# Meng-333/FastDiffSR

Measured on AMD Instinct MI355X. Metric: 256x256 SR images/sec at T=20, higher is better.
Workload: dtype f16x3; 1 GPU; x4 64->256, batch=16/GPU, T=20, random-init FastDiffSR UNet (inner 64, mults 1-2-4-4), 256x256, conv arithmetic f16x3 (BASELINE configs[1]); batch_per_gpu=16, global_batch=16, noise=drawn in the loop by the engine (Philox4x32-10), hipgraph=False, parallelism=dp1 (independent batches, weights broadcast once)

## Files before the change

fastdiffsr_amd/csrc/fdsr_conv_k32.hip:

```cpp
#include "fdsr_kernels.h"
#include "fdsr_act_io.h"

#include <type_traits>

namespace fdsr {

typedef float k_f32x4 __attribute__((ext_vector_type(4)));
typedef _Float16 k_h8 __attribute__((ext_vector_type(8)));
typedef _Float16 k_h4 __attribute__((ext_vector_type(4)));
typedef __bf16 k_b8 __attribute__((ext_vector_type(8)));
typedef __bf16 k_b4 __attribute__((ext_vector_type(4)));

__device__ __forceinline__ float silu_k(float v) { return v * __builtin_amdgcn_rcpf(1.0f + __expf(-v)); }

#ifndef XS_F16X3
#define XS_F16X3 2
#endif
#ifndef XS_BF16
#define XS_BF16 4
#endif
#ifndef K32_PIN
#define K32_PIN 1
#endif
#ifndef K32_RIDER2
#define K32_RIDER2 1
#endif
#ifndef K32_SPLIT
#define K32_SPLIT 1
#endif
#ifndef K32_SPLIT_BF16
#define K32_SPLIT_BF16 1
#endif
#ifndef K32_MIXSPLIT
#define K32_MIXSPLIT 1
#endif
#ifndef K32_PEEL
#define K32_PEEL 1
#endif
#ifndef K32_GNB_DIAG
#define K32_GNB_DIAG 0
#endif
#ifndef K32_DIAG
#define K32_DIAG 0
#endif
#ifndef K32_RFIRST
#define K32_RFIRST 1
#endif
#ifndef K32_PIN16
#define K32_PIN16 0
#endif

constexpr int K32_GNC_MAXC = 1024, K32_GNC_MAXP = K32_GNC_MAXC / 2 + 32, K32_GNC_LDS = K32_GNC_MAXP * 32 + K32_GNC_MAXC * 8;

template <int TH, int WN, int PREC, int NW_ = 8>
struct ConvK32Cfg {
  static constexpr int TW = 32, NW = NW_, KC = 32;
  static constexpr int NP = PREC == PREC_F16X3 ? 2 : 1;
  static constexpr int WNP = PREC == PREC_BF16 ? 1 : 2;
  static constexpr int ROWB = 64 * NP;
  static constexpr int HH = TH + 2, HWD = TW + 2, NPIX = HH * HWD;
  static constexpr int WM = NW / WN, BN = 32 * WN, MB = TH / WM;
  static constexpr int NT = 64 * NW;
  static constexpr int Q4 = KC / 4;
  static constexpr int RPP = NT / Q4;
  static constexpr int NIN = (NPIX + RPP - 1) / RPP;
  static constexpr int BUF_BYTES = NPIX * ROWB;
  static constexpr int LDS_BYTES = 2 * BUF_BYTES;
  static constexpr int R = 3;
  static constexpr int XS = PREC == PREC_F16X3 ? XS_F16X3 : (NW_ == 4 && TH == 8 ? 3 : XS_BF16);
  static_assert(MB == 4 || MB == 3 || MB == 2, "wave tile = 4 (small grids: 2; small workgroups in f16x3: 3) rows of 32 pixels");
  static_assert(((TH - WM + 2) * HWD + 16) * ROWB < 65536, "fragment offsets must fit the ds_read immediate");
};

template <int PREC>
__device__ __forceinline__ int k32_slot(int slot, int hx) {
  return PREC == PREC_F16X3 ? (slot ^ (hx & 7)) : (slot ^ ((hx >> 1) & 3));
}

template <int TH, int WN, int PREC, bool RIDER, int NW = 8, bool RF = (NW == 4), bool GNB = false, bool DROP = false, bool GNC = false>
__global__ void __launch_bounds__(64 * NW, 2) conv_k32_kernel(const ConvParams p) {
  using Cfg = ConvK32Cfg<TH, WN, PREC, NW>;
  constexpr int TW = Cfg::TW, KC = Cfg::KC, NP = Cfg::NP, ROWB = Cfg::ROWB, HWD = Cfg::HWD, NPIX = Cfg::NPIX;
  constexpr int WM = Cfg::WM, BN = Cfg::BN, MB = Cfg::MB, RPP = Cfg::RPP, NIN = Cfg::NIN, R = Cfg::R, XS = Cfg::XS;
  constexpr bool PIN = TH == 16 ? K32_PIN16 != 0 : K32_PIN != 0;

  extern __shared__ __attribute__((aligned(16))) unsigned char smem_k[];
  unsigned char* sBuf0 = smem_k;
  unsigned char* sBuf1 = smem_k + Cfg::BUF_BYTES;
  const int Cin = p.C0 + p.C1;

  const int tid = threadIdx.x, lane = tid & 63, wave = tid >> 6;
  const int wn = wave % WN, wm = wave / WN;
  const int c15 = lane & 15, g = lane >> 4;

  const int nco = p.Cout_pad / BN;
  const int tilesX = (p.Wout + TW - 1) / TW, tilesY = (p.Hout + TH - 1) / TH;
  int bid;
  {
    const int nwg = gridDim.x, b = blockIdx.x;
    const int q8 = nwg >> 3, r8 = nwg & 7, xcd = b & 7, k = b >> 3;
    bid = (xcd < r8 ? xcd * (q8 + 1) : r8 * (q8 + 1) + (xcd - r8) * q8) + k;
  }
  const int SK = p.ksplit > 1 ? p.ksplit : 1;
  const int ksi = bid % SK;
  bid /= SK;
  const int cot = bid % nco;
  int pt = bid / nco;
  const int tx = pt % tilesX;
  pt /= tilesX;
  const int ty = pt % tilesY;
  const int n = pt / tilesY;
  const int oy0 = ty * TH, ox0 = tx * TW, co0 = cot * BN;

  const bool gn = GNC ? true : p.gn_scale != nullptr;

  if (NW == 4 && p.stagger > 0) {
    unsigned hwid;
    asm volatile("s_getreg_b32 %0, hwreg(HW_REG_HW_ID)" : "=s"(hwid));
    if ((hwid >> 16) & 1u) {
      const int n64 = p.stagger * (p.Cin_pad / KC + (RIDER ? p.nkr / 2 : 0));
      for (int i = 0; i < n64; i += 8) __builtin_amdgcn_s_sleep(8);
    }
  }

  const int q = tid & 7, row0 = tid >> 3;
  int in_pix[NIN];
  unsigned long long skeys = 0;
  static_assert(NIN <= 21, "swizzle keys are packed into one register pair");
#pragma unroll
  for (int i = 0; i < NIN; ++i) {
    const int pix = row0 + i * RPP;
    int v = -2;
    if (pix < NPIX) {
      const int hy = pix / HWD, hx = pix % HWD;
      const int iy = oy0 - 1 + hy, ix = ox0 - 1 + hx;
      const bool ok = iy >= 0 && iy < p.Hin && ix >= 0 && ix < p.Win;
      v = ok ? (n * p.Hin + iy) * p.Win + ix : -1;
      skeys |= (unsigned long long)k32_slot<PREC>(0, hx) << (3 * i);
    }
    in_pix[i] = v;
  }
  const int sbase = row0 * ROWB + 8 * (q & 1);

  using IO = ActIO<PREC>;
  typedef typename IO::Quad Quad;
  struct QM { Quad q; unsigned m; };
  constexpr bool RFIRST = RIDER && RF && K32_RFIRST != 0;
  constexpr bool SPLIT = K32_SPLIT != 0 && (PREC == PREC_F16X3 || K32_SPLIT_BF16 != 0) && (!RIDER || RFIRST);
  static_assert(!RFIRST || SPLIT, "the rider-first path writes whole chunks into rr1, which is sized for them only when SPLIT");
  constexpr int NA = SPLIT ? (NIN + 1) / 2 : NIN;
  typedef std::integral_constant<int, 0> I_0;
  typedef std::integral_constant<int, NA> I_A;
  typedef std::integral_constant<int, NIN> I_N;
  QM rin[NA];
  QM rr1[RIDER && SPLIT ? NIN : 1];
  QM rin2[RIDER && K32_RIDER2 && NW == 8 ? NIN : 1];
  k_f32x4 rsc = {1.f, 1.f, 1.f, 1.f}, rsh = {0.f, 0.f, 0.f, 0.f};
  const int nk = p.Cin_pad / KC;
  const int nk16 = p.Cin_pad / 16;
  const int nkr = RIDER ? p.nkr / 2 : 0;
  double* gnc_pr = reinterpret_cast<double*>(smem_k + Cfg::LDS_BYTES);
  float* gnc_sc = reinterpret_cast<float*>(smem_k + Cfg::LDS_BYTES + K32_GNC_MAXP * 32);
  float* gnc_sh = gnc_sc + K32_GNC_MAXC;
  int gnc_lo = 0, gnc_hi = 0, gnc_cpg = 1, gnc_q0 = 0, gnc_q1 = 0;
  constexpr int GNC_PT = (2 * K32_GNC_MAXP + Cfg::NT - 1) / Cfg::NT;
  uint4 gnc_ld[GNC ? GNC_PT : 1][GSUM_SHARDS / 2];
  constexpr int GNC_CT = (K32_GNC_MAXC + Cfg::NT - 1) / Cfg::NT;
  float gnc_gam[GNC ? GNC_CT : 1], gnc_bet[GNC ? GNC_CT : 1];
  auto gnc_issue = [&](int c_lo, int c_hi) __attribute__((always_inline)) {
    gnc_lo = c_lo; gnc_hi = c_hi;
    gnc_cpg = Cin / p.gs_G;
    gnc_q0 = (c_lo / gnc_cpg) * gnc_cpg / 2;
    gnc_q1 = ((c_hi - 1) / gnc_cpg + 1) * gnc_cpg / 2;
#pragma unroll
    for (int j = 0; j < GNC_PT; ++j) {
      const int u = tid + j * Cfg::NT, qc = min(gnc_q0 + (u >> 1), gnc_q1 - 1);
      const bool first = qc < (p.C0 >> 1);
      const unsigned long long* tab = first ? p.gs0 : p.gs1;
      const int np = (first ? p.C0 : p.C1) >> 1, ql = first ? qc : qc - (p.C0 >> 1);
#pragma unroll
      for (int sdx = 0; sdx < GSUM_SHARDS / 2; ++sdx)
        gnc_ld[j][sdx] = *reinterpret_cast<const uint4*>(tab + (((size_t)n * GSUM_SHARDS + (u & 1) * (GSUM_SHARDS / 2) + sdx) * np + ql) * 2);
    }
#pragma unroll
    for (int j = 0; j < GNC_CT; ++j) {
      const int cc = min(c_lo + tid + j * Cfg::NT, c_hi - 1);
      gnc_gam[j] = p.gs_gamma[cc];
      gnc_bet[j] = p.gs_beta[cc];
    }
  };
  auto gnc_finish = [&]() __attribute__((always_inline)) {
#pragma unroll
    for (int j = 0; j < GNC_PT; ++j) {
      const int u = tid + j * Cfg::NT, qi = gnc_q0 + (u >> 1);
      long long a = 0, b = 0;
#pragma unroll
      for (int sdx = 0; sdx < GSUM_SHARDS / 2; ++sdx) {
        a += (long long)(((unsigned long long)gnc_ld[j][sdx].y << 32) | gnc_ld[j][sdx].x);
        b += (long long)(((unsigned long long)gnc_ld[j][sdx].w << 32) | gnc_ld[j][sdx].z);
      }
      if (qi < gnc_q1) {
        gnc_pr[2 * u] = (double)a * (1.0 / (double)(1 << GSUM_BITS1));
        gnc_pr[2 * u + 1] = (double)b * (1.0 / (double)(1 << GSUM_BITS2));
      }
    }
    __syncthreads();
    const double inv = 1.0 / ((double)gnc_cpg * (double)p.Hin * (double)p.Win);
#pragma unroll
    for (int j = 0; j < GNC_CT; ++j) {
      const int c = gnc_lo + tid + j * Cfg::NT;
      if (c >= gnc_hi) break;
      const int g = c / gnc_cpg, hp = gnc_cpg >> 1;
      double s1 = 0.0, s2 = 0.0;
      for (int k = 0; k < 2 * hp; ++k) { s1 += gnc_pr[2 * (2 * (g * hp - gnc_q0) + k)]; s2 += gnc_pr[2 * (2 * (g * hp - gnc_q0) + k) + 1]; }
      const double mean = s1 * inv;
      double var = s2 * inv - mean * mean;
      var = var < 0.0 ? 0.0 : var;
      const double rstd = 1.0 / sqrt(var + (double)p.gs_eps);
      const float scv = (float)rstd * gnc_gam[j];
      gnc_sc[c - gnc_lo] = scv;
      gnc_sh[c - gnc_lo] = gnc_bet[j] - (float)mean * scv;
    }
    __syncthreads();
  };
  auto prefetch_rng = [&](int kc, QM* rin, auto i0_tag, auto i1_tag, bool load_gn) __attribute__((always_inline)) {
    constexpr int I0 = decltype(i0_tag)::value, I1 = decltype(i1_tag)::value;
    int cbase = kc * KC;
    const float* base;
    int Cs, cc;
    bool gg = gn;
    if (RIDER && kc >= nk) {
      cbase -= nk * KC;
      gg = false;
      if (cbase < p.Cr0) { base = p.xr0; Cs = p.Cr0; cc = cbase + q * 4; }
      else { base = p.xr1; Cs = p.Cr1; cc = cbase - p.Cr0 + q * 4; }
    } else if (cbase < p.C0) { base = p.x0; Cs = p.C0; cc = cbase + q * 4; }
    else { base = p.x1; Cs = p.C1; cc = cbase - p.C0 + q * 4; }
    if (!GNC && gg && load_gn) {
      rsc = *reinterpret_cast<const k_f32x4*>(p.gn_scale + (size_t)n * Cin + cbase + q * 4);
      rsh = *reinterpret_cast<const k_f32x4*>(p.gn_shift + (size_t)n * Cin + cbase + q * 4);
    }
#pragma unroll
    for (int i = I0; i < I1; ++i) {
      const size_t pi = (size_t)(in_pix[i] < 0 ? 0 : in_pix[i]);
      rin[i - I0].q = IO::load4(base, pi * Cs + cc);
      if (DROP)
        rin[i - I0].m = *reinterpret_cast<const unsigned*>(p.drop_mask + ((RIDER && kc >= nk) ? (size_t)0 : pi * Cs + cc));
    }
  };
  auto prefetch_to = [&](int kc, QM* rin) __attribute__((always_inline)) { prefetch_rng(kc, rin, I_0{}, I_N{}, true); };
  auto stage_rng = [&](int kc, unsigned char* buf, const QM* rin, auto i0_tag, auto i1_tag) __attribute__((always_inline)) {
    constexpr int I0 = decltype(i0_tag)::value, I1 = decltype(i1_tag)::value;
    k_f32x4 sc = rsc, sh = rsh;
    if (GNC && !(RIDER && kc >= nk)) {
      sc = *reinterpret_cast<const k_f32x4*>(gnc_sc + (kc * KC - gnc_lo + q * 4));
      sh = *reinterpret_cast<const k_f32x4*>(gnc_sh + (kc * KC - gnc_lo + q * 4));
    }
#pragma unroll
    for (int i = I0; i < I1; ++i) {
      if (NIN * RPP > NPIX && i == NIN - 1 && row0 + i * RPP >= NPIX) continue;
      k_f32x4 v = IO::widen(rin[i - I0].q);
      if (K32_DIAG & 16) v = sc;
      if ((K32_DIAG & 1) && gn) {
        v = v + sh;
      } else if (gn && !(RIDER && kc >= nk)) {
        v = v * sc + sh;
        if (!p.gn_plain) { v.x = silu_k(v.x); v.y = silu_k(v.y); v.z = silu_k(v.z); v.w = silu_k(v.w); }
        if (DROP) {
          const unsigned m = rin[i - I0].m;
#pragma unroll
          for (int e = 0; e < 4; ++e) v[e] *= (float)((m >> (8 * e)) & 0xffu) * p.drop_scale;
        }
      } else if (PREC == PREC_F16X3 && p.sat_flag) {
        sat_check(p.sat_flag, v, 65504.f);
      }
      const int sd = sbase + i * (RPP * ROWB) + 16 * ((q >> 1) ^ (int)((skeys >> (3 * i)) & 7u));
      unsigned char* dst = buf + sd;
      if (PREC == PREC_F16X3) {
        const float lim = in_pix[i] >= 0 ? 65504.f : 0.f;
#pragma unroll
        for (int e = 0; e < 4; ++e) v[e] = __builtin_amdgcn_fmed3f(v[e], -lim, lim);
#if K32_MIXSPLIT
        typedef _Float16 h2t __attribute__((ext_vector_type(2)));
        uint2 hi, lo;
        {
          const h2t h0 = {(_Float16)v[0], (_Float16)v[1]}, h1 = {(_Float16)v[2], (_Float16)v[3]};
          hi.x = __builtin_bit_cast(unsigned, h0);
          hi.y = __builtin_bit_cast(unsigned, h1);
        }
        asm("v_fma_mixlo_f16 %0, %1, -1.0, %2 op_sel:[0,0,0] op_sel_hi:[1,0,0]" : "=v"(lo.x) : "v"(hi.x), "v"(v[0]));
        asm("v_fma_mixhi_f16 %0, %1, -1.0, %2 op_sel:[1,0,0] op_sel_hi:[1,0,0]" : "+v"(lo.x) : "v"(hi.x), "v"(v[1]));
        asm("v_fma_mixlo_f16 %0, %1, -1.0, %2 op_sel:[0,0,0] op_sel_hi:[1,0,0]" : "=v"(lo.y) : "v"(hi.y), "v"(v[2]));
        asm("v_fma_mixhi_f16 %0, %1, -1.0, %2 op_sel:[1,0,0] op_sel_hi:[1,0,0]" : "+v"(lo.y) : "v"(hi.y), "v"(v[3]));
        *reinterpret_cast<uint2*>(dst) = hi;
        *reinterpret_cast<uint2*>(buf + (sd ^ 64)) = lo;
#else
        k_h4 hi = {(_Float16)v.x, (_Float16)v.y, (_Float16)v.z, (_Float16)v.w};
        k_h4 lo = {(_Float16)(v.x - (float)hi.x), (_Float16)(v.y - (float)hi.y), (_Float16)(v.z - (float)hi.z),
                   (_Float16)(v.w - (float)hi.w)};
        *reinterpret_cast<k_h4*>(dst) = hi;
        *reinterpret_cast<k_h4*>(buf + (sd ^ 64)) = lo;
#endif
      } else {
        const float keep = in_pix[i] >= 0 ? 1.f : 0.f;
        v = v * keep;
        const uint2 hb = stage4_16<PREC>(v);
        if (K32_DIAG & 8) asm volatile("" ::"v"(hb.x), "v"(hb.y));
        else *reinterpret_cast<uint2*>(dst) = hb;
      }
    }
  };
  auto stage_from = [&](int kc, unsigned char* buf, const QM* rin) __attribute__((always_inline)) { stage_rng(kc, buf, rin, I_0{}, I_N{}); };

  const uint4* wq = reinterpret_cast<const uint4*>(p.wq);
  const int nkt = RIDER ? nk + nkr : nk;
  uint4 Wf[R][2][NP];
  const int wlane = 32 * (g & 1) + c15;
  auto load_w = [&](int kc, int tap, int slot) __attribute__((always_inline)) {
    if (K32_DIAG & 32) kc = 0;
    const uint4* src = wq + ((((size_t)cot * nk16 + 2 * kc + (g >> 1)) * WN + wn) * 9 + tap) * (Cfg::WNP * 64) + wlane;
    if (RIDER && kc >= nk)
      src = reinterpret_cast<const uint4*>(p.wq_r) + (((size_t)cot * p.nkr + 2 * (kc - nk) + (g >> 1)) * WN + wn) * (Cfg::WNP * 64) + wlane;
#pragma unroll
    for (int ch = 0; ch < 2; ++ch)
#pragma unroll
      for (int pl = 0; pl < NP; ++pl) Wf[slot][ch][pl] = src[pl * 64 + 16 * ch];
  };

  int xoff[3][NP];
#pragma unroll
  for (int kx = 0; kx < 3; ++kx) {
    const int hx = c15 + kx;
    xoff[kx][0] = (wm * HWD + hx) * ROWB + 16 * k32_slot<PREC>(g, hx);
    if (NP == 2) xoff[kx][NP - 1] = xoff[kx][0] ^ 64;
  }

  k_f32x4 acc[MB][2][2];
#pragma unroll
  for (int mb = 0; mb < MB; ++mb)
#pragma unroll
// ... 197 lines not shown
#pragma unroll
      for (int pl = 0; pl < NP; ++pl) xptr[1][pl] = cur + xoff[1][pl];
#pragma unroll
      for (int mb = 0; mb < XS - 1 && mb < MB; ++mb) load_x(mb, 1, 1, mb);
#pragma unroll
      for (int mb = 0; mb < MB; ++mb) {
        if (mb + XS - 1 < MB) load_x((mb + XS - 1) % XS, 1, 1, mb + XS - 1);
        mfma_step(mb % XS, 0, mb);
      }
      if (kc + 1 < kc1) {
        load_w(kc + 1, 0, 0);
        stage_from(kc + 1, nxt, r1);
        if (kc + 1 + AH < kc1) prefetch_to(kc + 1 + AH, r1);
      }
      __syncthreads();
    };
    QM* rfirst = SPLIT ? rr1 : rin;
    if (AH == 2) {
      for (int kc = k0; kc < kc1; kc += 2) {
        rider_chunk(kc, rfirst);
        if (kc + 1 < kc1) rider_chunk(kc + 1, rin2);
      }
    } else {
      for (int kc = k0; kc < kc1; ++kc) rider_chunk(kc, rfirst);
    }
  }

  k_f32x4 add[2];
  bool cok[2];
  const float* tembp = p.temb ? p.temb + (size_t)n * p.temb_stride + p.temb_off : p.bias;
  const float tmul = p.temb ? 1.f : 0.f;
#pragma unroll
  for (int ch = 0; ch < 2; ++ch) {
    const int co = cob + 16 * ch;
    cok[ch] = co < p.Cout;
    const int cs = cok[ch] ? co : 0;
#pragma unroll
    for (int r = 0; r < 4; ++r) {
      float a = p.bias[cs + r];
      if (RIDER) a += p.bias_r[cs + r];
      a += tmul * tembp[cs + r];
      add[ch][r] = a;
    }
  }
  const float winv_m = p.w_inv_scale_dev ? *p.w_inv_scale_dev : p.w_inv_scale;
  const float winv = RIDER && !RFIRST ? (p.w_inv_scale_r_dev ? *p.w_inv_scale_r_dev : p.w_inv_scale_r) : winv_m;
  if (RIDER && !RFIRST && kc1 <= nk) {
    const float ratio = winv_m / winv;
#pragma unroll
    for (int mb = 0; mb < MB; ++mb)
#pragma unroll
      for (int ph = 0; ph < 2; ++ph)
#pragma unroll
        for (int ch = 0; ch < 2; ++ch) acc[mb][ph][ch] *= ratio;
  }
  if (SK > 1) {
    float* sb = p.kscratch + (size_t)ksi * p.N * p.Hout * p.Wout * p.Cout;
#pragma unroll
    for (int mb = 0; mb < MB; ++mb)
#pragma unroll
      for (int ph = 0; ph < 2; ++ph)
#pragma unroll
        for (int ch = 0; ch < 2; ++ch) {
          const int oy = oy0 + wm + mb * WM, ox = ox0 + 16 * ph + c15;
          if (interior || (cok[ch] && oy < p.Hout && ox < p.Wout))
            *reinterpret_cast<k_f32x4*>(sb + obase + mb * rstride + ph * pstride + 16 * ch) = acc[mb][ph][ch];
        }
    return;
  }
  k_f32x4 s1[2], s2[2];
#pragma unroll
  for (int ch = 0; ch < 2; ++ch) s1[ch] = s2[ch] = k_f32x4{0.f, 0.f, 0.f, 0.f};
  auto epilogue = [&](auto out16_tag) __attribute__((always_inline)) {
    constexpr bool OUT16 = decltype(out16_tag)::value;
    auto put4 = [&](size_t idx, k_f32x4 v) {
      if (OUT16) {
        *reinterpret_cast<uint2*>(reinterpret_cast<unsigned short*>(p.out) + idx) = pack4_16<PREC>(v);
      } else {
        *reinterpret_cast<k_f32x4*>(p.out + idx) = v;
      }
    };
    if (interior) {
      if (p.res && !res_early) {
#pragma unroll
        for (int mb = 0; mb < MB; ++mb)
#pragma unroll
          for (int ph = 0; ph < 2; ++ph)
#pragma unroll
            for (int ch = 0; ch < 2; ++ch) rv[mb][ph][ch] = IO::load4(p.res, obase + mb * rstride + ph * pstride + 16 * ch);
      }
#pragma unroll
      for (int mb = 0; mb < MB; ++mb)
#pragma unroll
        for (int ph = 0; ph < 2; ++ph)
#pragma unroll
          for (int ch = 0; ch < 2; ++ch) {
            k_f32x4 v = acc[mb][ph][ch] * winv + add[ch];
            if (p.res) v += IO::widen(rv[mb][ph][ch]);
            put4(obase + mb * rstride + ph * pstride + 16 * ch, v);
            if (!(K32_DIAG & 4)) {
              s1[ch] += v;
              s2[ch] += v * v;
            }
          }
    } else {
#pragma unroll
      for (int mb = 0; mb < MB; ++mb)
#pragma unroll
        for (int ph = 0; ph < 2; ++ph)
#pragma unroll
          for (int ch = 0; ch < 2; ++ch) {
            const int oy = oy0 + wm + mb * WM, ox = ox0 + 16 * ph + c15;
            if (cok[ch] && oy < p.Hout && ox < p.Wout) {
              const size_t idx = obase + mb * rstride + ph * pstride + 16 * ch;
              k_f32x4 v = acc[mb][ph][ch] * winv + add[ch];
              if (p.res) v += IO::widen(IO::load4(p.res, idx));
              put4(idx, v);
              s1[ch] += v;
              s2[ch] += v * v;
            }
          }
    }
  };
  auto epilogue_gnb = [&](auto int_tag) __attribute__((always_inline)) {
    constexpr bool INTERIOR = decltype(int_tag)::value;
    const int Ct = p.Cout, cpg = Ct / p.gb_G;
    const bool hm = p.gb_mask != nullptr;
    const unsigned char* mk = hm ? p.gb_mask : reinterpret_cast<const unsigned char*>(p.gb_scale);
    const float ds = p.gb_drop;
#pragma unroll
    for (int ch = 0; ch < 2; ++ch) {
      const int cs = cok[ch] ? cob + 16 * ch : 0;
      const k_f32x4 gsc = *reinterpret_cast<const k_f32x4*>(p.gb_scale + (size_t)n * Ct + cs);
      const k_f32x4 gsh = *reinterpret_cast<const k_f32x4*>(p.gb_shift + (size_t)n * Ct + cs);
      k_f32x4 gme, grs;
#pragma unroll
      for (int r = 0; r < 4; ++r) {
        const int grp = (cs + r) / cpg;
        gme[r] = p.gb_stats[((size_t)n * p.gb_G + grp) * 2];
        grs[r] = p.gb_stats[((size_t)n * p.gb_G + grp) * 2 + 1];
      }
      const float* xb;
      int xcs;
      if (cs < p.gb_C0) { xb = p.gb_x0 + cs; xcs = p.gb_C0; }
      else { xb = p.gb_x1 + (cs - p.gb_C0); xcs = Ct - p.gb_C0; }
      k_f32x4 xq[MB][2];
      unsigned mq[MB][2];
#pragma unroll
      for (int mb = 0; mb < MB; ++mb) {
        const int oy = min(oy0 + wm + mb * WM, p.Hout - 1);
#pragma unroll
        for (int ph = 0; ph < 2; ++ph) {
          const size_t pix = (size_t)(n * p.Hout + oy) * p.Wout + min(ox0 + 16 * ph + c15, p.Wout - 1);
          if (K32_GNB_DIAG & 2) { xq[mb][ph] = gsc; mq[mb][ph] = 0x01010101u; continue; }
          xq[mb][ph] = *reinterpret_cast<const k_f32x4*>(xb + pix * xcs);
          mq[mb][ph] = *reinterpret_cast<const unsigned*>(mk + (hm ? pix * Ct + cs : (size_t)0));
        }
      }
#pragma unroll
      for (int mb = 0; mb < MB; ++mb) {
        const int oy = oy0 + wm + mb * WM;
#pragma unroll
        for (int ph = 0; ph < 2; ++ph) {
          const int ox = ox0 + 16 * ph + c15;
          const bool ok = INTERIOR || (cok[ch] && oy < p.Hout && ox < p.Wout);
          const k_f32x4 v = acc[mb][ph][ch] * winv + add[ch];
          const k_f32x4 x = xq[mb][ph];
          const unsigned m = mq[mb][ph];
          k_f32x4 gq, gx;
#pragma unroll
          for (int r = 0; r < 4; ++r) {
            float d = v[r];
            if (hm) d = ((m >> (8 * r)) & 0xffu) ? d * ds : 0.f;
            const float xh = (x[r] - gme[r]) * grs[r];
            float gg = d;
            if (!p.gb_plain && !(K32_GNB_DIAG & 1)) {
              const float u = fmaf(x[r], gsc[r], gsh[r]);
              const float sg = __builtin_amdgcn_rcpf(1.0f + __expf(-u));
              gg = d * (sg * (1.0f + u * (1.0f - sg)));
            }
            gq[r] = gg;
            gx[r] = gg * xh;
          }
          if (ok) {
            *reinterpret_cast<k_f32x4*>(p.out + obase + mb * rstride + ph * pstride + 16 * ch) = gq;
            s1[ch] += gq;
            s2[ch] += gx;
          }
        }
      }
    }
  };
  if constexpr (GNB) {
    if (interior) epilogue_gnb(std::true_type{});
    else epilogue_gnb(std::false_type{});
  } else {
    if (prec_is16(PREC) && !p.out_f32) epilogue(std::true_type{});
    else epilogue(std::false_type{});
  }
  if (p.part_out) {
    float vals[16];
#pragma unroll
    for (int ch = 0; ch < 2; ++ch)
#pragma unroll
      for (int r = 0; r < 4; ++r) { vals[ch * 8 + r * 2] = s1[ch][r]; vals[ch * 8 + r * 2 + 1] = s2[ch][r]; }
#pragma unroll
    for (int half = 8; half >= 1; half >>= 1) {
      const bool up = (c15 & half) != 0;
#pragma unroll
      for (int i = 0; i < half; ++i) {
        const float keep = up ? vals[i + half] : vals[i];
        const float send = up ? vals[i] : vals[i + half];
        vals[i] = keep + __shfl_xor(send, half, 64);
      }
    }
    float* sp = reinterpret_cast<float*>(smem_k);
    {
      const int ch = c15 >> 3, r = (c15 >> 1) & 3, st = c15 & 1;
      sp[(wm * BN + wn * 32 + 16 * ch + 4 * g + r) * 2 + st] = vals[0];
    }
    __syncthreads();
    float a_keep = 0.f, b_keep = 0.f;
    if (tid < BN && co0 + tid < p.Cout) {
      float a = 0.f, b = 0.f;
#pragma unroll
      for (int w = 0; w < WM; ++w) { a += sp[(w * BN + tid) * 2 + 0]; b += sp[(w * BN + tid) * 2 + 1]; }
      a_keep = a; b_keep = b;
      float* dst = p.part_out + (((size_t)n * (tilesX * tilesY) + ty * tilesX + tx) * p.Cout + co0 + tid) * 2;
      dst[0] = a;
      dst[1] = b;
    }
    if (p.gsum_out) {
      const float a2 = a_keep + __shfl_xor(a_keep, 1, 64), b2 = b_keep + __shfl_xor(b_keep, 1, 64);
      if (tid < BN && !(tid & 1) && co0 + tid < p.Cout) gsum_add(p.gsum_out, n, p.Cout >> 1, (co0 + tid) >> 1, xcc_id(), a2, b2);
    }
  }
}

template <int TH, int WN, int PREC>
struct ConvUp2K32Cfg {
  static constexpr int TW = 32, KC = 32;
  static constexpr int NP = PREC == PREC_F16X3 ? 2 : 1;
  static constexpr int WNP = PREC == PREC_BF16 ? 1 : 2;
  static constexpr int ROWB = 64 * NP;
  static constexpr int HH = TH + 1, HWD = TW + 2, NPIX = HH * HWD;
  static constexpr int WM = 8 / WN, BN = 32 * WN, MB = TH / WM;
  static constexpr int RPP = 512 / 8, NIN = (NPIX + RPP - 1) / RPP;
  static constexpr int BUF_BYTES = NPIX * ROWB;
  static constexpr int R = 4;
  static_assert(MB == 2, "two source rows per wave");
};

template <int TH, int WN, int PREC>
__global__ void __launch_bounds__(512, 2) conv_up2_k32_kernel(const ConvParams p) {
  using Cfg = ConvUp2K32Cfg<TH, WN, PREC>;
  constexpr int TW = Cfg::TW, KC = Cfg::KC, NP = Cfg::NP, ROWB = Cfg::ROWB, HWD = Cfg::HWD, NPIX = Cfg::NPIX;
  constexpr int WM = Cfg::WM, BN = Cfg::BN, MB = Cfg::MB, RPP = Cfg::RPP, NIN = Cfg::NIN, R = Cfg::R;

  extern __shared__ __attribute__((aligned(16))) unsigned char smem_uk[];
  unsigned char* sBuf0 = smem_uk;
  unsigned char* sBuf1 = smem_uk + Cfg::BUF_BYTES;

  const int tid = threadIdx.x, lane = tid & 63, wave = tid >> 6;
  const int wn = wave % WN, wm = wave / WN;
  const int c15 = lane & 15, g = lane >> 4;

  const int nco = p.Cout_pad / BN;
  const int tilesX = (p.Win + TW - 1) / TW, tilesY = (p.Hin + TH - 1) / TH;
  int bid;
  {
    const int nwg = gridDim.x, b = blockIdx.x;
    const int q8 = nwg >> 3, r8 = nwg & 7, xcd = b & 7, k = b >> 3;
    bid = (xcd < r8 ? xcd * (q8 + 1) : r8 * (q8 + 1) + (xcd - r8) * q8) + k;
  }
  const int cot = bid % nco;
  int pt = bid / nco;
  const int py = pt & 1;
  pt >>= 1;
  const int tx = pt % tilesX;
  pt /= tilesX;
  const int ty = pt % tilesY;
  const int n = pt / tilesY;
  const int oy0 = ty * TH, ox0 = tx * TW, co0 = cot * BN;

  const int q = tid & 7, row0 = tid >> 3;
  int in_pix[NIN];
  unsigned skeys = 0;
#pragma unroll
  for (int i = 0; i < NIN; ++i) {
    const int pix = row0 + i * RPP;
    int v = -2;
    if (pix < NPIX) {
      const int hy = pix / HWD, hx = pix % HWD;
      const int iy = oy0 - 1 + py + hy, ix = ox0 - 1 + hx;
      const bool ok = iy >= 0 && iy < p.Hin && ix >= 0 && ix < p.Win;
      v = ok ? (n * p.Hin + iy) * p.Win + ix : -1;
      skeys |= (unsigned)k32_slot<PREC>(0, hx) << (3 * i);
    }
    in_pix[i] = v;
  }
  const int sbase = row0 * ROWB + 8 * (q & 1);
  using IO = ActIO<PREC>;
  typedef typename IO::Quad Quad;
  Quad rin[NIN];
  auto prefetch = [&](int kc) {
    const size_t coff = (size_t)kc * KC + q * 4;
#pragma unroll
    for (int i = 0; i < NIN; ++i) rin[i] = IO::load4(p.x0, (size_t)(in_pix[i] < 0 ? 0 : in_pix[i]) * p.C0 + coff);
  };
  auto stage = [&](unsigned char* buf) {
#pragma unroll
    for (int i = 0; i < NIN; ++i) {
      if (NIN * RPP > NPIX && i == NIN - 1 && row0 + i * RPP >= NPIX) continue;
      k_f32x4 v = IO::widen(rin[i]);
      const int sd = sbase + i * (RPP * ROWB) + 16 * ((q >> 1) ^ (int)((skeys >> (3 * i)) & 7u));
      if (PREC == PREC_F16X3) {
        if (p.sat_flag) sat_check(p.sat_flag, v, 65504.f);
        const float lim = in_pix[i] >= 0 ? 65504.f : 0.f;
#pragma unroll
        for (int e = 0; e < 4; ++e) v[e] = __builtin_amdgcn_fmed3f(v[e], -lim, lim);
        typedef _Float16 h2t __attribute__((ext_vector_type(2)));
        uint2 hi, lo;
        {
          const h2t h0 = {(_Float16)v[0], (_Float16)v[1]}, h1 = {(_Float16)v[2], (_Float16)v[3]};
          hi.x = __builtin_bit_cast(unsigned, h0);
          hi.y = __builtin_bit_cast(unsigned, h1);
        }
        asm("v_fma_mixlo_f16 %0, %1, -1.0, %2 op_sel:[0,0,0] op_sel_hi:[1,0,0]" : "=v"(lo.x) : "v"(hi.x), "v"(v[0]));
        asm("v_fma_mixhi_f16 %0, %1, -1.0, %2 op_sel:[1,0,0] op_sel_hi:[1,0,0]" : "+v"(lo.x) : "v"(hi.x), "v"(v[1]));
        asm("v_fma_mixlo_f16 %0, %1, -1.0, %2 op_sel:[0,0,0] op_sel_hi:[1,0,0]" : "=v"(lo.y) : "v"(hi.y), "v"(v[2]));
        asm("v_fma_mixhi_f16 %0, %1, -1.0, %2 op_sel:[1,0,0] op_sel_hi:[1,0,0]" : "+v"(lo.y) : "v"(hi.y), "v"(v[3]));
        *reinterpret_cast<uint2*>(buf + sd) = hi;
        *reinterpret_cast<uint2*>(buf + (sd ^ 64)) = lo;
      } else {
        const float keep = in_pix[i] >= 0 ? 1.f : 0.f;
        v = v * keep;
        *reinterpret_cast<uint2*>(buf + sd) = stage4_16<PREC>(v);
      }
    }
  };

  const uint4* wq = reinterpret_cast<const uint4*>(p.wq);
  const int nk = p.Cin_pad / KC, nk16 = p.Cin_pad / 16;
  uint4 Wf[R][2][NP];
  const int wlane = 32 * (g & 1) + c15;
  auto load_w = [&](int kc, int slot) {
    const uint4* src = wq + ((((((size_t)cot * nk16 + 2 * kc + (g >> 1)) * WN + wn) * 2 + py) * 8 + slot) * (Cfg::WNP * 64)) + wlane;
#pragma unroll
    for (int ch = 0; ch < 2; ++ch)
#pragma unroll
      for (int pl = 0; pl < NP; ++pl) Wf[slot % R][ch][pl] = src[pl * 64 + 16 * ch];
  };

  int xoff[3][NP];
#pragma unroll
  for (int c = 0; c < 3; ++c) {
    const int hx = c15 + c;
    xoff[c][0] = (wm * HWD + hx) * ROWB + 16 * k32_slot<PREC>(g, hx);
    if (NP == 2) xoff[c][NP - 1] = xoff[c][0] ^ 64;
  }

  k_f32x4 acc[MB][2][2][2];
#pragma unroll
  for (int mb = 0; mb < MB; ++mb)
#pragma unroll
    for (int px = 0; px < 2; ++px)
#pragma unroll
      for (int ph = 0; ph < 2; ++ph)
#pragma unroll
        for (int ch = 0; ch < 2; ++ch) acc[mb][px][ph][ch] = k_f32x4{0.f, 0.f, 0.f, 0.f};

#pragma unroll
  for (int sl = 0; sl < R; ++sl) load_w(0, sl);
  prefetch(0);
  stage(sBuf0);
  if (nk > 1) prefetch(1);
  __syncthreads();

  uint4 Xf[2][2][NP];
  const unsigned char* xptr[3][NP];
  auto load_x = [&](int xs, int slot, int mb) {
    const int a = (slot >> 1) & 1, c = (slot >> 2) + (slot & 1);
#pragma unroll
    for (int ph = 0; ph < 2; ++ph)
#pragma unroll
      for (int pl = 0; pl < NP; ++pl)
        Xf[xs][ph][pl] = *reinterpret_cast<const uint4*>(xptr[c][pl] + ((mb * WM + a) * HWD + 16 * ph) * ROWB);
  };
  auto mfma_step = [&](int xs, int slot, int mb) {
    const int px = slot >> 2, ws = slot % R;
    if (PREC == PREC_F16X3) {
#pragma unroll
      for (int term = 0; term < 3; ++term)
#pragma unroll
        for (int ph = 0; ph < 2; ++ph)
#pragma unroll
          for (int ch = 0; ch < 2; ++ch) {
            const uint4 xv = Xf[xs][ph][term == 0 ? NP - 1 : 0];
            const uint4 wv = Wf[ws][ch][term == 1 ? NP - 1 : 0];
            acc[mb][px][ph][ch] = __builtin_amdgcn_mfma_f32_16x16x32_f16(__builtin_bit_cast(k_h8, wv), __builtin_bit_cast(k_h8, xv),
                                                                        acc[mb][px][ph][ch], 0, 0, 0);
          }
    } else {
#pragma unroll
      for (int ph = 0; ph < 2; ++ph)
#pragma unroll
        for (int ch = 0; ch < 2; ++ch)
          acc[mb][px][ph][ch] = mfma16_k32<PREC>(Wf[ws][ch][0], Xf[xs][ph][0], acc[mb][px][ph][ch]);
    }
  };

  for (int kc = 0; kc < nk; ++kc) {
    unsigned char* cur = (kc & 1) ? sBuf1 : sBuf0;
    unsigned char* nxt = (kc & 1) ? sBuf0 : sBuf1;
    const bool more = kc + 1 < nk;
#pragma unroll
    for (int c = 0; c < 3; ++c)
#pragma unroll
      for (int pl = 0; pl < NP; ++pl) xptr[c][pl] = cur + xoff[c][pl];
    load_x(0, 0, 0);
#pragma unroll
    for (int slot = 0; slot < 8; ++slot) {
#pragma unroll
      for (int mb = 0; mb < MB; ++mb) {
        const int s = slot * MB + mb;
        if (s + 1 < 8 * MB) load_x((s + 1) & 1, (s + 1) / MB, (s + 1) % MB);
        __builtin_amdgcn_sched_barrier(0);
        mfma_step(s & 1, slot, mb);
        __builtin_amdgcn_sched_barrier(0);
      }
      if (slot + R < 8) load_w(kc, slot + R);
      else if (more) load_w(kc + 1, slot + R - 8);
      if (slot == 3 && more) {
        stage(nxt);
        if (kc + 2 < nk) prefetch(kc + 2);
      }
    }
    __syncthreads();
  }

  const int cob = co0 + wn * 32 + 4 * g;
  const float winv = p.w_inv_scale_dev ? *p.w_inv_scale_dev : p.w_inv_scale;
  k_f32x4 add[2];
  bool cok[2];
  const float* tembp = p.temb ? p.temb + (size_t)n * p.temb_stride + p.temb_off : p.bias;
  const float tmul = p.temb ? 1.f : 0.f;
#pragma unroll
  for (int ch = 0; ch < 2; ++ch) {
    const int co = cob + 16 * ch;
    cok[ch] = co < p.Cout;
    const int cs = cok[ch] ? co : 0;
#pragma unroll
    for (int r = 0; r < 4; ++r) add[ch][r] = p.bias[cs + r] + tmul * tembp[cs + r];
  }
  k_f32x4 s1[2], s2[2];
#pragma unroll
  for (int ch = 0; ch < 2; ++ch) s1[ch] = s2[ch] = k_f32x4{0.f, 0.f, 0.f, 0.f};
  const bool out16 = prec_is16(PREC);
#pragma unroll
  for (int mb = 0; mb < MB; ++mb)
#pragma unroll
    for (int px = 0; px < 2; ++px)
#pragma unroll
      for (int ph = 0; ph < 2; ++ph)
#pragma unroll
        for (int ch = 0; ch < 2; ++ch) {
          const int sy = oy0 + wm + mb * WM, sx = ox0 + 16 * ph + c15;
          if (cok[ch] && sy < p.Hin && sx < p.Win) {
            const size_t idx = ((size_t)(n * p.Hout + 2 * sy + py) * p.Wout + 2 * sx + px) * p.Cout + cob + 16 * ch;
            const k_f32x4 v = acc[mb][px][ph][ch] * winv + add[ch];
            if (out16) {
              *reinterpret_cast<uint2*>(reinterpret_cast<unsigned short*>(p.out) + idx) = pack4_16<PREC>(v);
            } else {
              *reinterpret_cast<k_f32x4*>(p.out + idx) = v;
            }
            s1[ch] += v;
            s2[ch] += v * v;
          }
        }
  if (p.part_out) {
    float vals[16];
#pragma unroll
    for (int ch = 0; ch < 2; ++ch)
#pragma unroll
      for (int r = 0; r < 4; ++r) { vals[ch * 8 + r * 2] = s1[ch][r]; vals[ch * 8 + r * 2 + 1] = s2[ch][r]; }
#pragma unroll
    for (int half = 8; half >= 1; half >>= 1) {
      const bool up = (c15 & half) != 0;
#pragma unroll
      for (int i = 0; i < half; ++i) {
        const float keep = up ? vals[i + half] : vals[i];
        const float send = up ? vals[i] : vals[i + half];
        vals[i] = keep + __shfl_xor(send, half, 64);
      }
    }
    float* sp = reinterpret_cast<float*>(smem_uk);
    {
      const int ch = c15 >> 3, r = (c15 >> 1) & 3, st = c15 & 1;
      sp[(wm * BN + wn * 32 + 16 * ch + 4 * g + r) * 2 + st] = vals[0];
    }
    __syncthreads();
    float a_keep = 0.f, b_keep = 0.f;
    if (tid < BN && co0 + tid < p.Cout) {
      float a = 0.f, b = 0.f;
#pragma unroll
      for (int w = 0; w < WM; ++w) { a += sp[(w * BN + tid) * 2 + 0]; b += sp[(w * BN + tid) * 2 + 1]; }
      a_keep = a; b_keep = b;
      float* dst = p.part_out + (((size_t)n * (tilesX * tilesY * 2) + (ty * tilesX + tx) * 2 + py) * p.Cout + co0 + tid) * 2;
      dst[0] = a;
      dst[1] = b;
    }
    if (p.gsum_out) {
      const float a2 = a_keep + __shfl_xor(a_keep, 1, 64), b2 = b_keep + __shfl_xor(b_keep, 1, 64);
      if (tid < BN && !(tid & 1) && co0 + tid < p.Cout) gsum_add(p.gsum_out, n, p.Cout >> 1, (co0 + tid) >> 1, xcc_id(), a2, b2);
    }
  }
}

bool conv_up2_k32_ok(int prec, const ConvParams& p) {
  if (!(g_tun.k32 & FDSR_K32_UP2) || !(g_tun.k32 & (prec_is16(prec) ? FDSR_K32_BF16 : FDSR_K32_F16X3))) return false;
  return p.C1 == 0 && p.C0 % 32 == 0 && p.C0 == p.Cin_pad && p.Cout % 4 == 0 && !p.gn_scale && !p.res;
}

template <int TH, int WN, int PREC>
static hipError_t launch_up2_k32_t(const ConvParams& q, int nwg, hipStream_t s) {
  using Cfg = ConvUp2K32Cfg<TH, WN, PREC>;
  hipLaunchKernelGGL((conv_up2_k32_kernel<TH, WN, PREC>), dim3(nwg), dim3(512), (size_t)2 * Cfg::BUF_BYTES, s, q);
  return hipGetLastError();
}

#define FDSR_UP2_K32_SHAPES(X) X(8, 2) X(4, 4) X(2, 8)

hipError_t launch_conv_up2_k32(int TH, int WN, int prec, const ConvParams& q, int nwg, hipStream_t s) {
#define X(TH_, WN_)                                                                                    \
  if (TH == TH_ && WN == WN_)                                                                          \
    return prec == PREC_F16X3 ? launch_up2_k32_t<TH_, WN_, PREC_F16X3>(q, nwg, s) : prec == PREC_F16 ? launch_up2_k32_t<TH_, WN_, PREC_F16>(q, nwg, s) : launch_up2_k32_t<TH_, WN_, PREC_BF16>(q, nwg, s);
  FDSR_UP2_K32_SHAPES(X)
#undef X
  return hipErrorInvalidValue;
}

#define FDSR_K32_SHAPES(X) X(16, 2) X(8, 4) X(4, 8) X(8, 2) X(4, 4) X(2, 8)

bool conv_k32_ok(int TH, int WN, int prec, const ConvParams& p) {
  if (!(g_tun.k32 & (prec_is16(prec) ? FDSR_K32_BF16 : FDSR_K32_F16X3))) return false;
  if (TH == 16 && p.xr0 && !(g_tun.k32 & FDSR_K32_RIDER_16ROW)) return false;
  if (TH * WN != 32 && !(TH * WN == 16 && (g_tun.k32 & FDSR_K32_SMALL_GRID_2ROW))) return false;
  if (WN != 2 && WN != 4 && WN != 8) return false;
  if (p.Cin_pad % 32 || (p.C0 + p.C1) != p.Cin_pad) return false;
  if (p.C1 != 0 && p.C0 % 32) return false;
  if (p.Cout % 4) return false;
  if (p.xr0) {
    if (p.nkr % 2 || (p.Cr0 + p.Cr1) != p.nkr * 16) return false;
    if (p.Cr1 != 0 && p.Cr0 % 32) return false;
  }
  return true;
}

template <int TH, int WN, int PREC, bool RIDER, int NW = 8, bool RF = (NW == 4), bool GNB = false, bool DROP = false, bool GNC = false>
static hipError_t launch_k32_t(const ConvParams& q, int nwg, hipStream_t s) {
  using Cfg = ConvK32Cfg<TH, WN, PREC, NW>;
  hipLaunchKernelGGL((conv_k32_kernel<TH, WN, PREC, RIDER, NW, RF, GNB, DROP, GNC>), dim3(nwg), dim3(Cfg::NT), (size_t)Cfg::LDS_BYTES + (GNC ? K32_GNC_LDS : 0), s, q);
  return hipGetLastError();
}

bool conv_k32_drop_ok(int prec, const ConvParams& q) {
  if (prec != PREC_F16X3 || !q.drop_mask || !q.gn_scale || q.gn_plain || q.C1 != 0 || q.ksplit > 1 || q.gb_x0) return false;
  return !q.xr0 || (g_tun.k32 & FDSR_K32_RIDER_FIRST_8WAVE);
}

static bool k32_gnb_ok(int prec, const ConvParams& q) {
  if (prec != PREC_F16X3 || !q.out_f32 || q.xr0 || q.res || q.ksplit > 1 || !q.gb_scale || !q.gb_shift || !q.gb_stats) return false;
  if (q.gb_G <= 0 || q.Cout % q.gb_G || q.Cout % 4) return false;
  return q.gb_x1 ? (q.gb_C0 % 4 == 0 && q.gb_C0 > 0 && q.gb_C0 < q.Cout) : q.gb_C0 == q.Cout;
}

static int k32_small_rows(int prec, bool rider) { return prec_is16(prec) && !rider ? 8 : 6; }

bool conv_k32_small_ok(ConvKind kind, int prec, const ConvParams& p) {
  if (!(g_tun.k32 & FDSR_K32_SMALL_WG_F16X3) || kind != CONV3_S1 || p.ksplit > 1 || p.Cout_pad != 64) return false;
  if (prec_is16(prec) && !(g_tun.k32 & FDSR_K32_SMALL_WG_BF16)) return false;
  if (p.xr0 && !(g_tun.k32 & (prec_is16(prec) ? FDSR_K32_SMALL_WG_RIDER_BF16 : FDSR_K32_SMALL_WG_RIDER_F16X3))) return false;
  if (!conv_k32_ok(8, 4, prec, p)) return false;
  const int th = k32_small_rows(prec, p.xr0 != nullptr);
  const long wgs = (long)p.N * ((p.Wout + 31) / 32) * ((p.Hout + th - 1) / th);
  return wgs >= g_tun.k32_sb_min_wgs;
}

hipError_t launch_conv_k32_small(int prec, const ConvParams& p, hipStream_t s, int* tiles) {
  const int th = k32_small_rows(prec, p.xr0 != nullptr);
  const int tilesX = (p.Wout + 31) / 32, tilesY = (p.Hout + th - 1) / th;
  if (tiles) *tiles = tilesX * tilesY;
  const int nwg = p.N * tilesX * tilesY;
  ConvParams q = p;
  q.out_bf16 = p.out_f32 ? 0 : prec_act16(prec);
  q.stagger = g_tun.k32_stagger;
  if (q.gb_x0) return k32_gnb_ok(prec, q) ? launch_k32_t<6, 2, PREC_F16X3, false, 4, true, true>(q, nwg, s) : hipErrorInvalidValue;
  if (q.drop_mask) {
    if (!conv_k32_drop_ok(prec, q)) return hipErrorInvalidValue;
    return q.xr0 ? launch_k32_t<6, 2, PREC_F16X3, true, 4, true, false, true>(q, nwg, s) : launch_k32_t<6, 2, PREC_F16X3, false, 4, true, false, true>(q, nwg, s);
  }
  if (prec == PREC_F16X3)
    return q.xr0 ? launch_k32_t<6, 2, PREC_F16X3, true, 4>(q, nwg, s) : launch_k32_t<6, 2, PREC_F16X3, false, 4>(q, nwg, s);
  if (prec == PREC_F16) return q.xr0 ? launch_k32_t<6, 2, PREC_F16, true, 4>(q, nwg, s) : launch_k32_t<8, 2, PREC_F16, false, 4>(q, nwg, s);
  return q.xr0 ? launch_k32_t<6, 2, PREC_BF16, true, 4>(q, nwg, s) : launch_k32_t<8, 2, PREC_BF16, false, 4>(q, nwg, s);
}

#define FDSR_K32_GNC_SHAPES(X) X(8, 2) X(4, 4) X(2, 8)
bool conv_k32_gnc_ok(int TH, int WN, int prec, const ConvParams& p) {
  if (TH * WN != 16 || !conv_k32_ok(TH, WN, prec, p)) return false;
  if (p.gb_x0 || p.drop_mask || p.gn_plain || (p.C0 & 1) || (p.C1 & 1)) return false;
  const int Cin = p.C0 + p.C1;
  return Cin <= K32_GNC_MAXC && p.gs_G > 0 && Cin % p.gs_G == 0 && ((Cin / p.gs_G) & 1) == 0;
}

hipError_t launch_conv_k32(int TH, int WN, int prec, const ConvParams& q, int nwg, hipStream_t s) {
  if (q.gs0) {
    if (!conv_k32_gnc_ok(TH, WN, prec, q)) return hipErrorInvalidValue;
    const bool rf = q.xr0 && q.ksplit <= 1 && (g_tun.k32 & FDSR_K32_RIDER_FIRST_8WAVE);
#define X(TH_, WN_)                                                                                                      \
    if (TH == TH_ && WN == WN_) {                                                                                        \
      if (rf) return prec == PREC_F16X3 ? launch_k32_t<TH_, WN_, PREC_F16X3, true, 8, true, false, false, true>(q, nwg, s)   \
                                        : prec == PREC_F16 ? launch_k32_t<TH_, WN_, PREC_F16, true, 8, true, false, false, true>(q, nwg, s) : launch_k32_t<TH_, WN_, PREC_BF16, true, 8, true, false, false, true>(q, nwg, s);    \
      if (q.xr0) return prec == PREC_F16X3 ? launch_k32_t<TH_, WN_, PREC_F16X3, true, 8, false, false, false, true>(q, nwg, s)  \
                                           : prec == PREC_F16 ? launch_k32_t<TH_, WN_, PREC_F16, true, 8, false, false, false, true>(q, nwg, s) : launch_k32_t<TH_, WN_, PREC_BF16, true, 8, false, false, false, true>(q, nwg, s);   \
      return prec == PREC_F16X3 ? launch_k32_t<TH_, WN_, PREC_F16X3, false, 8, false, false, false, true>(q, nwg, s)      \
                                : prec == PREC_F16 ? launch_k32_t<TH_, WN_, PREC_F16, false, 8, false, false, false, true>(q, nwg, s) : launch_k32_t<TH_, WN_, PREC_BF16, false, 8, false, false, false, true>(q, nwg, s);       \
    }
    FDSR_K32_GNC_SHAPES(X)
#undef X
    return hipErrorInvalidValue;
  }
#define X(TH_, WN_)                                                                                             \
  if (TH == TH_ && WN == WN_) {                                                                                 \
    if (q.gb_x0) return k32_gnb_ok(prec, q) ? launch_k32_t<TH_, WN_, PREC_F16X3, false, 8, false, true>(q, nwg, s) : hipErrorInvalidValue; \
    if (q.drop_mask) {                                                                                          \
      if (!conv_k32_drop_ok(prec, q)) return hipErrorInvalidValue;                                              \
      return q.xr0 ? launch_k32_t<TH_, WN_, PREC_F16X3, true, 8, true, false, true>(q, nwg, s)                  \
                   : launch_k32_t<TH_, WN_, PREC_F16X3, false, 8, false, false, true>(q, nwg, s);               \
    }                                                                                                           \
    if (q.xr0 && q.ksplit <= 1 && (g_tun.k32 & FDSR_K32_RIDER_FIRST_8WAVE))                                                           \
      return prec == PREC_F16X3 ? launch_k32_t<TH_, WN_, PREC_F16X3, true, 8, true>(q, nwg, s)                  \
                                : prec == PREC_F16 ? launch_k32_t<TH_, WN_, PREC_F16, true, 8, true>(q, nwg, s) : launch_k32_t<TH_, WN_, PREC_BF16, true, 8, true>(q, nwg, s);                  \
    if (q.xr0) return prec == PREC_F16X3 ? launch_k32_t<TH_, WN_, PREC_F16X3, true>(q, nwg, s)                  \
                                         : prec == PREC_F16 ? launch_k32_t<TH_, WN_, PREC_F16, true>(q, nwg, s) : launch_k32_t<TH_, WN_, PREC_BF16, true>(q, nwg, s);                  \
    return prec == PREC_F16X3 ? launch_k32_t<TH_, WN_, PREC_F16X3, false>(q, nwg, s)                            \
                              : prec == PREC_F16 ? launch_k32_t<TH_, WN_, PREC_F16, false>(q, nwg, s) : launch_k32_t<TH_, WN_, PREC_BF16, false>(q, nwg, s);                            \
  }
  FDSR_K32_SHAPES(X)
#undef X
  return hipErrorInvalidValue;
}

template <int TH, int WN, int PREC, bool RIDER, int NW = 8, bool RF = (NW == 4), bool GNB = false, bool DROP = false, bool GNC = false>
static hipError_t init_k32_t() {
  auto kfn = conv_k32_kernel<TH, WN, PREC, RIDER, NW, RF, GNB, DROP, GNC>;
  return hipFuncSetAttribute(reinterpret_cast<const void*>(kfn), hipFuncAttributeMaxDynamicSharedMemorySize, 160 * 1024);
}

template <int TH, int WN, int PREC>
static hipError_t init_up2_k32_t() {
  auto kfn = conv_up2_k32_kernel<TH, WN, PREC>;
  return hipFuncSetAttribute(reinterpret_cast<const void*>(kfn), hipFuncAttributeMaxDynamicSharedMemorySize, 160 * 1024);
}

hipError_t kernels_k32_init() {
  hipError_t e;
#define X(TH_, WN_)                                                                 \
  if ((e = init_up2_k32_t<TH_, WN_, PREC_F16X3>()) != hipSuccess) return e;         \
  if ((e = init_up2_k32_t<TH_, WN_, PREC_BF16>()) != hipSuccess) return e; \
  if ((e = init_up2_k32_t<TH_, WN_, PREC_F16>()) != hipSuccess) return e;
  FDSR_UP2_K32_SHAPES(X)
#undef X
#define X(TH_, WN_)                                                                        \
  if ((e = init_k32_t<TH_, WN_, PREC_F16X3, false>()) != hipSuccess) return e;             \
  if ((e = init_k32_t<TH_, WN_, PREC_F16X3, true>()) != hipSuccess) return e;              \
  if ((e = init_k32_t<TH_, WN_, PREC_BF16, false>()) != hipSuccess) return e;              \
  if ((e = init_k32_t<TH_, WN_, PREC_F16, false>()) != hipSuccess) return e;              \
  if ((e = init_k32_t<TH_, WN_, PREC_BF16, true>()) != hipSuccess) return e;                \
  if ((e = init_k32_t<TH_, WN_, PREC_F16, true>()) != hipSuccess) return e;                \
  if ((e = init_k32_t<TH_, WN_, PREC_F16X3, true, 8, true>()) != hipSuccess) return e;     \
  if ((e = init_k32_t<TH_, WN_, PREC_F16X3, false, 8, false, true>()) != hipSuccess) return e; \
  if ((e = init_k32_t<TH_, WN_, PREC_F16X3, false, 8, false, false, true>()) != hipSuccess) return e; \
  if ((e = init_k32_t<TH_, WN_, PREC_F16X3, true, 8, true, false, true>()) != hipSuccess) return e; \
  if ((e = init_k32_t<TH_, WN_, PREC_BF16, true, 8, true>()) != hipSuccess) return e; \
  if ((e = init_k32_t<TH_, WN_, PREC_F16, true, 8, true>()) != hipSuccess) return e;
  FDSR_K32_SHAPES(X)
#undef X
#define X(TH_, WN_)                                                                                                     \
  if ((e = init_k32_t<TH_, WN_, PREC_F16X3, false, 8, false, false, false, true>()) != hipSuccess) return e;            \
  if ((e = init_k32_t<TH_, WN_, PREC_F16X3, true, 8, false, false, false, true>()) != hipSuccess) return e;             \
  if ((e = init_k32_t<TH_, WN_, PREC_F16X3, true, 8, true, false, false, true>()) != hipSuccess) return e;              \
  if ((e = init_k32_t<TH_, WN_, PREC_BF16, false, 8, false, false, false, true>()) != hipSuccess) return e;             \
  if ((e = init_k32_t<TH_, WN_, PREC_F16, false, 8, false, false, false, true>()) != hipSuccess) return e;             \
  if ((e = init_k32_t<TH_, WN_, PREC_BF16, true, 8, false, false, false, true>()) != hipSuccess) return e;              \
  if ((e = init_k32_t<TH_, WN_, PREC_F16, true, 8, false, false, false, true>()) != hipSuccess) return e;              \
  if ((e = init_k32_t<TH_, WN_, PREC_BF16, true, 8, true, false, false, true>()) != hipSuccess) return e; \
  if ((e = init_k32_t<TH_, WN_, PREC_F16, true, 8, true, false, false, true>()) != hipSuccess) return e;
  FDSR_K32_GNC_SHAPES(X)
#undef X
  if ((e = init_k32_t<6, 2, PREC_F16X3, false, 4>()) != hipSuccess) return e;
  if ((e = init_k32_t<6, 2, PREC_F16X3, true, 4>()) != hipSuccess) return e;
  if ((e = init_k32_t<6, 2, PREC_F16X3, false, 4, true, true>()) != hipSuccess) return e;
  if ((e = init_k32_t<6, 2, PREC_F16X3, false, 4, true, false, true>()) != hipSuccess) return e;
  if ((e = init_k32_t<6, 2, PREC_F16X3, true, 4, true, false, true>()) != hipSuccess) return e;
  if ((e = init_k32_t<6, 2, PREC_BF16, true, 4>()) != hipSuccess) return e;
  if ((e = init_k32_t<6, 2, PREC_F16, true, 4>()) != hipSuccess) return e;
  return hipSuccess;
}

}
```

Measured before the change: 72.37 images/s.

## Peel last K chunk and hoist epilogue loads in upsample-fused conv kernel

Restructures the 2x-upsample conv kernel's main loop into a chunk lambda so the last K chunk is peeled. Bias and temb loads for the epilogue are issued during that final chunk, which hides their latency behind MFMA work. Interior tiles get a store path with no bounds checks. An optional split of the staging and prefetch into two halves is added but is off by default; peeling adds code size and register pressure.

Result: no change. 72.07 images/s (-0.4%).

```diff
diff --git a/fastdiffsr_amd/csrc/fdsr_conv_k32.hip b/fastdiffsr_amd/csrc/fdsr_conv_k32.hip
--- a/fastdiffsr_amd/csrc/fdsr_conv_k32.hip
+++ b/fastdiffsr_amd/csrc/fdsr_conv_k32.hip
@@ -36,6 +36,15 @@
 #endif
 #ifndef K32_PEEL
 #define K32_PEEL 1
+#endif
+#ifndef K32_UP2_SPLIT
+#define K32_UP2_SPLIT 0
+#endif
+#ifndef K32_UP2_SPLIT_16
+#define K32_UP2_SPLIT_16 0
+#endif
+#ifndef K32_UP2_PEEL
+#define K32_UP2_PEEL 1
 #endif
 #ifndef K32_GNB_DIAG
 #define K32_GNB_DIAG 0
@@ -839,17 +848,25 @@
   const int sbase = row0 * ROWB + 8 * (q & 1);
   using IO = ActIO<PREC>;
   typedef typename IO::Quad Quad;
-  Quad rin[NIN];
-  auto prefetch = [&](int kc) {
+  constexpr bool SPLIT = K32_UP2_SPLIT != 0 && (PREC == PREC_F16X3 || K32_UP2_SPLIT_16 != 0);
+  constexpr bool PEEL = K32_UP2_PEEL != 0;
+  constexpr int NA = SPLIT ? (NIN + 1) / 2 : NIN;
+  typedef std::integral_constant<int, 0> I_0;
+  typedef std::integral_constant<int, NA> I_A;
+  typedef std::integral_constant<int, NIN> I_N;
+  Quad rin[NA];
+  auto prefetch_rng = [&](int kc, Quad* r, auto i0_tag, auto i1_tag) __attribute__((always_inline)) {
+    constexpr int I0 = decltype(i0_tag)::value, I1 = decltype(i1_tag)::value;
     const size_t coff = (size_t)kc * KC + q * 4;
 #pragma unroll
-    for (int i = 0; i < NIN; ++i) rin[i] = IO::load4(p.x0, (size_t)(in_pix[i] < 0 ? 0 : in_pix[i]) * p.C0 + coff);
-  };
-  auto stage = [&](unsigned char* buf) {
-#pragma unroll
-    for (int i = 0; i < NIN; ++i) {
+    for (int i = I0; i < I1; ++i) r[i - I0] = IO::load4(p.x0, (size_t)(in_pix[i] < 0 ? 0 : in_pix[i]) * p.C0 + coff);
+  };
+  auto stage_rng = [&](unsigned char* buf, const Quad* r, auto i0_tag, auto i1_tag) __attribute__((always_inline)) {
+    constexpr int I0 = decltype(i0_tag)::value, I1 = decltype(i1_tag)::value;
+#pragma unroll
+    for (int i = I0; i < I1; ++i) {
       if (NIN * RPP > NPIX && i == NIN - 1 && row0 + i * RPP >= NPIX) continue;
-      k_f32x4 v = IO::widen(rin[i]);
+      k_f32x4 v = IO::widen(r[i - I0]);
       const int sd = sbase + i * (RPP * ROWB) + 16 * ((q >> 1) ^ (int)((skeys >> (3 * i)) & 7u));
       if (PREC == PREC_F16X3) {
         if (p.sat_flag) sat_check(p.sat_flag, v, 65504.f);
@@ -909,9 +926,18 @@
 
 #pragma unroll
   for (int sl = 0; sl < R; ++sl) load_w(0, sl);
-  prefetch(0);
-  stage(sBuf0);
-  if (nk > 1) prefetch(1);
+  if (SPLIT) {
+    {
+      Quad r0[NIN];
+      prefetch_rng(0, r0, I_0{}, I_N{});
+      stage_rng(sBuf0, r0, I_0{}, I_N{});
+    }
+    prefetch_rng(nk > 1 ? 1 : 0, rin, I_0{}, I_A{});
+  } else {
+    prefetch_rng(0, rin, I_0{}, I_N{});
+    stage_rng(sBuf0, rin, I_0{}, I_N{});
+    if (nk > 1) prefetch_rng(1, rin, I_0{}, I_N{});
+  }
   __syncthreads();
 
   uint4 Xf[2][2][NP];
@@ -947,15 +973,31 @@
     }
   };
 
-  for (int kc = 0; kc < nk; ++kc) {
+  const int cob = co0 + wn * 32 + 4 * g;
+  const float winv = p.w_inv_scale_dev ? *p.w_inv_scale_dev : p.w_inv_scale;
+  const float* tembp = p.temb ? p.temb + (size_t)n * p.temb_stride + p.temb_off : p.bias;
+  const float tmul = p.temb ? 1.f : 0.f;
+  bool cok[2];
+  k_f32x4 bia[2], tem[2];
+  auto load_add = [&](int ch) __attribute__((always_inline)) {
+    const int co = cob + 16 * ch;
+    cok[ch] = co < p.Cout;
+    const int cs = cok[ch] ? co : 0;
+#pragma unroll
+    for (int r = 0; r < 4; ++r) { bia[ch][r] = p.bias[cs + r]; tem[ch][r] = tembp[cs + r]; }
+  };
+
+  auto chunk = [&](int kc, auto last_tag) __attribute__((always_inline)) {
+    constexpr bool LAST = decltype(last_tag)::value;
     unsigned char* cur = (kc & 1) ? sBuf1 : sBuf0;
     unsigned char* nxt = (kc & 1) ? sBuf0 : sBuf1;
-    const bool more = kc + 1 < nk;
+    const bool more = LAST ? false : (PEEL ? true : kc + 1 < nk);
 #pragma unroll
     for (int c = 0; c < 3; ++c)
 #pragma unroll
       for (int pl = 0; pl < NP; ++pl) xptr[c][pl] = cur + xoff[c][pl];
     load_x(0, 0, 0);
+    if (LAST) load_add(0);
 #pragma unroll
     for (int slot = 0; slot < 8; ++slot) {
 #pragma unroll
@@ -968,42 +1010,54 @@
       }
       if (slot + R < 8) load_w(kc, slot + R);
       else if (more) load_w(kc + 1, slot + R - 8);
-      if (slot == 3 && more) {
-        stage(nxt);
-        if (kc + 2 < nk) prefetch(kc + 2);
-      }
+      if (SPLIT) {
+        if (slot == 2 && more) {
+          stage_rng(nxt, rin, I_0{}, I_A{});
+          prefetch_rng(kc + 1, rin, I_A{}, I_N{});
+        }
+        if (slot == 6 && more) {
+          stage_rng(nxt, rin, I_A{}, I_N{});
+          if (PEEL || kc + 2 < nk) prefetch_rng(kc + 2 < nk ? kc + 2 : nk - 1, rin, I_0{}, I_A{});
+        }
+      } else if (slot == 3 && more) {
+        stage_rng(nxt, rin, I_0{}, I_N{});
+        if (kc + 2 < nk) prefetch_rng(kc + 2, rin, I_0{}, I_N{});
+      }
+      if (LAST && slot == 4) load_add(1);
     }
     __syncthreads();
-  }
-
-  const int cob = co0 + wn * 32 + 4 * g;
-  const float winv = p.w_inv_scale_dev ? *p.w_inv_scale_dev : p.w_inv_scale;
+  };
+  if (PEEL) {
+    for (int kc = 0; kc < nk - 1; ++kc) chunk(kc, std::false_type{});
+    chunk(nk - 1, std::true_type{});
+  } else {
+    for (int kc = 0; kc < nk; ++kc) chunk(kc, std::false_type{});
+    load_add(0);
+    load_add(1);
+  }
+
   k_f32x4 add[2];
-  bool cok[2];
-  const float* tembp = p.temb ? p.temb + (size_t)n * p.temb_stride + p.temb_off : p.bias;
-  const float tmul = p.temb ? 1.f : 0.f;
-#pragma unroll
-  for (int ch = 0; ch < 2; ++ch) {
-    const int co = cob + 16 * ch;
-    cok[ch] = co < p.Cout;
-    const int cs = cok[ch] ? co : 0;
-#pragma unroll
-    for (int r = 0; r < 4; ++r) add[ch][r] = p.bias[cs + r] + tmul * tembp[cs + r];
-  }
+#pragma unroll
+  for (int ch = 0; ch < 2; ++ch)
+#pragma unroll
+    for (int r = 0; r < 4; ++r) add[ch][r] = bia[ch][r] + tmul * tem[ch][r];
   k_f32x4 s1[2], s2[2];
 #pragma unroll
   for (int ch = 0; ch < 2; ++ch) s1[ch] = s2[ch] = k_f32x4{0.f, 0.f, 0.f, 0.f};
   const bool out16 = prec_is16(PREC);
-#pragma unroll
-  for (int mb = 0; mb < MB; ++mb)
-#pragma unroll
-    for (int px = 0; px < 2; ++px)
-#pragma unroll
-      for (int ph = 0; ph < 2; ++ph)
-#pragma unroll
-        for (int ch = 0; ch < 2; ++ch) {
-          const int sy = oy0 + wm + mb * WM, sx = ox0 + 16 * ph + c15;
-          if (cok[ch] && sy < p.Hin && sx < p.Win) {
+  const bool interior = (oy0 + TH <= p.Hin) && (ox0 + TW <= p.Win) && (co0 + BN <= p.Cout);
+  auto store_tile = [&](auto int_tag) __attribute__((always_inline)) {
+    constexpr bool INTERIOR = decltype(int_tag)::value;
+#pragma unroll
+    for (int mb = 0; mb < MB; ++mb)
+#pragma unroll
+      for (int px = 0; px < 2; ++px)
+#pragma unroll
+        for (int ph = 0; ph < 2; ++ph)
+#pragma unroll
+          for (int ch = 0; ch < 2; ++ch) {
+            const int sy = oy0 + wm + mb * WM, sx = ox0 + 16 * ph + c15;
+            if (!INTERIOR && !(cok[ch] && sy < p.Hin && sx < p.Win)) continue;
             const size_t idx = ((size_t)(n * p.Hout + 2 * sy + py) * p.Wout + 2 * sx + px) * p.Cout + cob + 16 * ch;
             const k_f32x4 v = acc[mb][px][ph][ch] * winv + add[ch];
             if (out16) {
@@ -1014,7 +1068,9 @@
             s1[ch] += v;
             s2[ch] += v * v;
           }
-        }
+  };
+  if (interior) store_tile(std::true_type{});
+  else store_tile(std::false_type{});
   if (p.part_out) {
     float vals[16];
 #pragma unroll
```
